# soedinglab/metaeuk

Hardware: AMD Instinct MI355X
Metric: prefilter+align ORF-fragments/sec (hits UNVERIFIED in this run: no CPU reference digest) (higher is better)
Workload: dtype packed i16 / i32 DP on u8 residues, i8 scores

## Files before the change

### metaeuk_amd/csrc/mk_align.hip

```cpp
#include "mk_align.hpp"
#include "mk_filters.hpp"
#include "mk_kernels.hpp"
#include "mk_limits.hpp"
#include "mk_segsort.hpp"
#include <algorithm>
#include <cmath>
#include <cstdlib>
#include <cstring>
#include <atomic>
#include <map>
#include <mutex>
#include <omp.h>

namespace mk {

namespace {

constexpr uint32_t KEY_CLS = 4096;
constexpr int SW_NBINCFG = SW_NCFG + 2;
constexpr uint32_t N_BINS = (uint32_t) SW_NBINCFG * KEY_CLS;
static_assert(SW_NCFG <= 16, "the bounds arrays keep 16 slots per kind");

__device__ __forceinline__ uint32_t len_class(uint32_t tLen) { return KEY_CLS - 1 - min(tLen >> 4, KEY_CLS - 1); }
__device__ __forceinline__ uint32_t sort_key(uint32_t qLen, uint32_t tLen) { return (uint32_t) sw_cfg_of(qLen) * KEY_CLS + len_class(tLen); }
// ... 41 lines not shown
    }
}

__global__ __launch_bounds__(256) void expand_pairs_kernel(AlignView V, const uint64_t *hitOff, const mk_hit *hits, uint64_t n,
                                                           SwJob *jobs, uint32_t *badTarget,
                                                           unsigned long long *work ) {
    helper_prio();
    __shared__ unsigned long long sWork[2 * SW_NCFG];
    for (int k = threadIdx.x; k < 2 * SW_NCFG; k += blockDim.x) sWork[k] = 0;
    __syncthreads();
    const uint64_t p = (uint64_t) blockIdx.x * blockDim.x + threadIdx.x;
    if (p < n) {
        uint32_t lo = 0, hi = V.n_queries;
        while (hi - lo > 1) { const uint32_t mid = (lo + hi) >> 1; if (hitOff[mid] <= p) lo = mid; else hi = mid; }
        const uint32_t q = lo, t = hits[p].seq_id;
        SwJob j;
        j.q_start = (uint32_t) V.q_off[q]; j.q_len = (uint32_t) (V.q_off[q + 1] - V.q_off[q]);
        if (t < V.n_targets) { j.t_start = V.t_off[t]; j.t_len = (uint32_t) (V.t_off[t + 1] - V.t_off[t]); }
        else { j.t_start = 0; j.t_len = 0; atomicMax(badTarget, (uint32_t) p + 1u); }
        j.q_step = 1; j.t_step = 1; j.slot = (uint32_t) p;
        jobs[p] = j;
        const int c = sw_cfg_of(j.q_len);
        atomicAdd(&sWork[2 * c], (unsigned long long) (j.t_len + 2u * j.q_len + (uint32_t) (sizeof(SwJob) + sizeof(SwOut))));
        atomicAdd(&sWork[2 * c + 1], (unsigned long long) j.q_len * j.t_len);
    }
    __syncthreads();
    for (int k = threadIdx.x; k < 2 * SW_NCFG; k += blockDim.x) if (sWork[k]) atomicAdd(&work[k], sWork[k]);
}

constexpr uint32_t ORDER_WAVE_MAX = 64, ORDER_TILE = 2048;
constexpr int PLAN_NV = 2 * SW_NCFG + 1;
constexpr uint32_t PLAN_BLOCK = 256;
struct PlanArgs {
    const uint64_t *hitOff; const uint64_t *q_off; uint32_t nq, nPairs; bool narrow;
    uint32_t *jobOff, *waveOff;
    uint32_t *runQuery, *runIndex;
    uint32_t *blockSums;
    uint32_t *bounds;
    uint32_t *waveStart;
};
__device__ __forceinline__ void plan_values(const PlanArgs &A, uint32_t q, uint32_t (&v)[PLAN_NV], int &cfg, uint32_t &n) {
#pragma unroll
    for (int k = 0; k < PLAN_NV; k++) v[k] = 0;
    cfg = 0; n = 0;
    if (q >= A.nq) return;
    n = (uint32_t) (A.hitOff[q + 1] - A.hitOff[q]);
    if (n == 0) return;
    cfg = sw_cfg_of((uint32_t) (A.q_off[q + 1] - A.q_off[q]));
    const uint32_t dpw = sw_cfg_jobs_per_wave(cfg, A.narrow);
#pragma unroll
    for (int c = 0; c < SW_NCFG; c++) if (c == cfg) { v[2 * c] = n; v[2 * c + 1] = (n + dpw - 1u) / dpw; }
    v[2 * SW_NCFG] = n > ORDER_WAVE_MAX ? (n + ORDER_TILE - 1u) / ORDER_TILE : 0u;
}
__global__ __launch_bounds__(PLAN_BLOCK) void plan_sums_kernel(PlanArgs A) {
    helper_prio();
    __shared__ uint32_t sm[PLAN_NV * 16];
    uint32_t v[PLAN_NV], excl[PLAN_NV], total[PLAN_NV], n;
    int cfg;
    plan_values(A, blockIdx.x * PLAN_BLOCK + threadIdx.x, v, cfg, n);
    segsort::block_scan<PLAN_NV>(v, excl, total, sm);
    if (threadIdx.x == 0)
#pragma unroll
        for (int k = 0; k < PLAN_NV; k++) A.blockSums[blockIdx.x * (PLAN_NV + 1) + k] = total[k];
}
__global__ __launch_bounds__(PLAN_BLOCK) void plan_offsets_kernel(PlanArgs A) {
    helper_prio();
    __shared__ uint32_t sm[PLAN_NV * 16];
    uint32_t v[PLAN_NV], w[PLAN_NV], excl[PLAN_NV], base[PLAN_NV], all[PLAN_NV], total[PLAN_NV], n;
#pragma unroll
    for (int k = 0; k < PLAN_NV; k++) { v[k] = 0; w[k] = 0; }
    for (uint32_t b = threadIdx.x; b < gridDim.x; b += PLAN_BLOCK)
#pragma unroll
        for (int k = 0; k < PLAN_NV; k++) {
            const uint32_t x = A.blockSums[b * (PLAN_NV + 1) + k];
            if (b < blockIdx.x) v[k] += x;
            w[k] += x;
        }
    segsort::block_scan<PLAN_NV>(v, excl, base, sm);
    segsort::block_scan<PLAN_NV>(w, excl, all, sm);
    const uint32_t q = blockIdx.x * PLAN_BLOCK + threadIdx.x;
    int cfg;
    plan_values(A, q, v, cfg, n);
    segsort::block_scan<PLAN_NV>(v, excl, total, sm);
    uint32_t jobBase = 0, waveBase = 0;
#pragma unroll
    for (int c = 0; c < SW_NCFG; c++) if (c < cfg) { jobBase += all[2 * c]; waveBase += all[2 * c + 1]; }
    if (q < A.nq) {
        uint32_t jo = jobBase, wo = waveBase;
#pragma unroll
        for (int c = 0; c < SW_NCFG; c++) if (c == cfg) { jo += base[2 * c] + excl[2 * c]; wo += base[2 * c + 1] + excl[2 * c + 1]; }
        A.jobOff[q] = jo; A.waveOff[q] = wo;
        const uint32_t runs = v[2 * SW_NCFG], r0 = base[2 * SW_NCFG] + excl[2 * SW_NCFG];
        for (uint32_t r = 0; r < runs; r++) { A.runQuery[r0 + r] = q; A.runIndex[r0 + r] = r; }
    }
    if (blockIdx.x == gridDim.x - 1 && threadIdx.x == 0) {
        uint32_t jb = 0, wb = 0;
        for (int c = 0; c < SW_NCFG; c++) { A.bounds[c] = jb; A.bounds[16 + c] = wb; jb += all[2 * c]; wb += all[2 * c + 1]; }
        A.bounds[SW_NCFG] = jb; A.bounds[16 + SW_NCFG] = wb; A.bounds[33] = all[2 * SW_NCFG];
        A.waveStart[wb] = A.nPairs;
    }
}
struct OrderArgs {
    const uint64_t *hitOff; const uint64_t *q_off; const mk_hit *hits; const uint64_t *t_off; uint32_t nq, nTargets; bool narrow;
    const uint32_t *jobOff, *waveOff, *runQuery, *runIndex;
    uint32_t *order, *waveStart;
};
__device__ __forceinline__ uint64_t order_key(const OrderArgs &A, uint64_t p) {
    const uint32_t t = A.hits[p].seq_id;
    const uint32_t tLen = t < A.nTargets ? (uint32_t) (A.t_off[t + 1] - A.t_off[t]) : 0u;
    return ((uint64_t) len_class(tLen) << 32) | (uint64_t) (uint32_t) p;
}
__global__ __launch_bounds__(256) void order_wave_kernel(OrderArgs A) {
    helper_prio();
    const uint32_t q = blockIdx.x * 4u + (threadIdx.x >> 6), lane = threadIdx.x & 63u;
    if (q >= A.nq) return;
    const uint64_t p0 = A.hitOff[q];
    const uint32_t n = (uint32_t) (A.hitOff[q + 1] - p0);
    if (n == 0 || n > ORDER_WAVE_MAX) return;
    const uint64_t key = lane < n ? order_key(A, p0 + lane) : ~0ull;
    const uint32_t r = segsort::wave_rank(key, n);
    const uint32_t jo = A.jobOff[q];
    if (lane < n) A.order[jo + r] = (uint32_t) (p0 + lane);
    const uint32_t dpw = sw_cfg_jobs_per_wave(sw_cfg_of((uint32_t) (A.q_off[q + 1] - A.q_off[q])), A.narrow);
    const uint32_t nW = (n + dpw - 1u) / dpw;
    if (lane < nW) A.waveStart[A.waveOff[q] + lane] = jo + lane * dpw;
}
__global__ __launch_bounds__(256) void order_block_kernel(OrderArgs A) {
    helper_prio();
    __shared__ uint64_t sK[ORDER_TILE];
    const uint32_t q = A.runQuery[blockIdx.x], run = A.runIndex[blockIdx.x];
    const uint64_t p0 = A.hitOff[q];
    const uint32_t n = (uint32_t) (A.hitOff[q + 1] - p0);
    const uint32_t b = run * ORDER_TILE, m = min(ORDER_TILE, n - b);
    const uint32_t P = segsort::pow2_at_least(m);
    for (uint32_t t = threadIdx.x; t < P; t += 256) sK[t] = t < m ? order_key(A, p0 + b + t) : ~0ull;
    __syncthreads();
    segsort::lds_sort<256>(sK, P);
    const uint32_t jo = A.jobOff[q] + b;
    for (uint32_t t = threadIdx.x; t < m; t += 256) A.order[jo + t] = (uint32_t) sK[t];
    const uint32_t dpw = sw_cfg_jobs_per_wave(sw_cfg_of((uint32_t) (A.q_off[q + 1] - A.q_off[q])), A.narrow);
    const uint32_t w0 = b / dpw, nW = (m + dpw - 1u) / dpw;
    for (uint32_t w = threadIdx.x; w < nW; w += 256) A.waveStart[A.waveOff[q] + w0 + w] = jo + w * dpw;
}
static_assert(ORDER_TILE % 8 == 0, "a run holds whole waves");

constexpr uint32_t SCAN_TILE = 1024;
__global__ __launch_bounds__(256) void scan_sums_kernel(const uint32_t *in, uint32_t n, uint32_t *blockSums) {
    helper_prio();
    __shared__ uint32_t sm[16];
    const uint32_t i0 = blockIdx.x * SCAN_TILE + threadIdx.x * 4u;
    uint32_t v[1] = {0}, excl[1], total[1];
#pragma unroll
    for (uint32_t k = 0; k < 4; k++) if (i0 + k < n) v[0] += in[i0 + k];
    segsort::block_scan<1>(v, excl, total, sm);
    if (threadIdx.x == 0) blockSums[blockIdx.x] = total[0];
}
__global__ __launch_bounds__(256) void scan_apply_kernel(const uint32_t *in, uint32_t n, uint32_t *out, const uint32_t *blockSums, uint32_t *grandTotal) {
    helper_prio();
    __shared__ uint32_t sm[16];
    uint32_t v[1] = {0}, excl[1], base[1], total[1];
    for (uint32_t b = threadIdx.x; b < blockIdx.x; b += 256) v[0] += blockSums[b];
    segsort::block_scan<1>(v, excl, base, sm);
    const uint32_t i0 = blockIdx.x * SCAN_TILE + threadIdx.x * 4u;
    uint32_t x[4];
    v[0] = 0;
#pragma unroll
    for (uint32_t k = 0; k < 4; k++) { x[k] = i0 + k < n ? in[i0 + k] : 0u; v[0] += x[k]; }
    segsort::block_scan<1>(v, excl, total, sm);
    uint32_t run = base[0] + excl[0];
#pragma unroll
    for (uint32_t k = 0; k < 4; k++) { if (i0 + k < n) out[i0 + k] = run; run += x[k]; }
    if (grandTotal && blockIdx.x == gridDim.x - 1 && threadIdx.x == 0) *grandTotal = base[0] + total[0];
}

__device__ __forceinline__ bool gate_pass(const SwJob *fwdJobs, const SwOut *fwdOut, uint64_t n, const GateEntry *gate, uint64_t p, SwJob &j) {
    if (p >= n) return false;
    const int score = fwdOut[p].score;
// ... 307 lines not shown
        for (int s = SCAN; s >= 1; s--) {
            const bool pass = !(eval(s) > evalThr);
            if (!pass) { lastFail = s; break; }
        }
        g.s0 = lastFail >= SCAN ? (1 << 30) : lastFail + 1;
        for (int s = 1; s < 256 && s < g.s0; s++)
            if (!(eval(s) > evalThr)) g.mask[s >> 5] |= 1u << (s & 31);
        table[L] = g;
    }
}

#define ACHK(x) do { hipError_t e_ = (x); if (e_ != hipSuccess) { err = std::string(#x) + ": " + hipGetErrorString(e_); return MK_ERR_DEVICE; } } while (0)
#define ANULL(p) do { if (!(p)) { err = "device scratch allocation failed (" #p ")"; return MK_ERR_DEVICE; } } while (0)

static int device_scan(const uint32_t *in, uint32_t n, uint32_t *out, uint32_t *total, hipStream_t stream, std::string &err) {
    if (n == 0) { if (total) ACHK(hipMemsetAsync(total, 0, 4, stream)); return MK_OK; }
    const uint32_t nb = (n + SCAN_TILE - 1u) / SCAN_TILE;
    uint32_t *sums = (uint32_t *) dev_scratch("align_scansums", (size_t) nb * 4);
    ANULL(sums);
    hipLaunchKernelGGL(scan_sums_kernel, dim3(nb), dim3(256), 0, stream, in, n, sums);
    hipLaunchKernelGGL(scan_apply_kernel, dim3(nb), dim3(256), 0, stream, in, n, out, (const uint32_t *) sums, total);
    ACHK(hipGetLastError());
    return MK_OK;
}

struct AlignShapes {
    int cus = 256;
    uint32_t persistentBlocks[SW_NCFG];
    uint32_t unitsPerBlock = 0;
    int knownForce = -1, knownWaves = 12;
    bool fwdLargeFirst = false;
    bool multiLargeFirst = true;
    bool multiPrio = true;
    uint32_t multiPerCu[3] = {24, 12, 12};
};
static bool sw_early_exit() { return knob_long("MK_SW_EARLY_EXIT", 1) != 0; }
static const AlignShapes &align_shapes() {
    static AlignShapes S;
    static std::once_flag once;
    std::call_once(once, [] {
        int dev = 0;
        (void) hipGetDevice(&dev);
        if (hipDeviceGetAttribute(&S.cus, hipDeviceAttributeMultiprocessorCount, dev) != hipSuccess || S.cus <= 0) S.cus = 256;
        int perCu[SW_NCFG];
        for (int c = 0; c < SW_NCFG; c++) perCu[c] = 12;
        if (const char *e = knob("MK_SW_WAVES_PER_CU")) {
            int k = 0, last = 16;
            for (const char *p = e; *p && k < SW_NCFG; k++) {
                last = std::max(1, atoi(p));
                perCu[k] = last;
                while (*p && *p != ',') p++;
                if (*p == ',') p++;
            }
            for (; k < SW_NCFG; k++) perCu[k] = last;
        }
        for (int c = 0; c < SW_NCFG; c++) S.persistentBlocks[c] = (uint32_t) (S.cus * perCu[c]);
        S.unitsPerBlock = (uint32_t) std::max(0L, knob_long("MK_SW_UNITS_PER_BLOCK", 0));
        S.knownForce = (int) knob_long("MK_SW_KNOWN", -1);
        S.knownWaves = (int) std::max(1L, knob_long("MK_SW_KNOWN_WAVES", 12));
        S.multiPrio = knob_long("MK_SW_MULTI_PRIO", 1) != 0;
        S.fwdLargeFirst = knob_long("MK_SW_FWD_LARGE_FIRST", 0) != 0;
        S.multiLargeFirst = knob_long("MK_SW_MULTI_LARGE_FIRST", 1) != 0;
        if (const char *e = knob("MK_SW_MULTI_WAVES")) {
            int k = 0;
            for (const char *p = e; *p && k < 3; k++) { S.multiPerCu[k] = (uint32_t) std::max(1, atoi(p)); while (*p && *p != ',') p++; if (*p == ',') p++; }
        }
    });
    return S;
}

static int tpos_first_cfg(const AlignView &V) {
    static_assert(SW_NCFG == 11, "configurations 8 / 9 = 512 / 768 rows");
    if (!V.q_prof || knob_long("MK_SW_TPOS", 1) == 0 || knob_long("MK_SW_MULTI", 0) != 0 || knob_long("MK_SW_NARROW", -1) == 0) return -1;
    return 8;
}

static int run_sorted_sw(const AlignView &V, const mk_params &P, const SwJob *jobs, SwOut *out, const uint32_t *keys, uint32_t *hist, uint32_t *order,
                         uint32_t n, const char *tag, hipStream_t stream, std::string &err,
                         timed_begin_fn tb, timed_end_fn te, int *handles ,
                         const int32_t *knownScore ) {
    if (handles) for (int c = 0; c < SW_NCFG; c++) handles[c] = -1;
    if (n == 0) return MK_OK;
    const AlignShapes &S = align_shapes();
    uint32_t *dCursor = (uint32_t *) dev_scratch("align_bincursor", (size_t) N_BINS * 4);
    uint32_t *dBounds = (uint32_t *) dev_scratch("align_bounds", 64 * sizeof(uint32_t));
    uint32_t *hb = (uint32_t *) pinned_scratch("align_bounds_h", 64 * sizeof(uint32_t));
    ANULL(dCursor); ANULL(dBounds); ANULL(hb);
    int th = tb("align_sort", 12.0 * n, 0);
    hipLaunchKernelGGL(bin_scan_kernel, dim3(1), dim3(BIN_THREADS), 0, stream, hist, dCursor, dBounds);
    hipLaunchKernelGGL(bin_scatter_kernel, dim3((n + 255) / 256), dim3(256), 0, stream, keys, n, dCursor, order);
// ... 70 lines not shown
        L.q_res = V.q_res; L.q_bias8 = V.q_bias8; L.q_prof = V.q_prof; L.t_res = V.t_res; L.mat = V.mat_aln;
        L.jobs = jobs; L.out = out; L.n_jobs = hi - lo; L.order = order + lo;
        L.boundary = nullptr; L.boundary_stride = 0; L.boundary_job0 = 0;
        L.wave_start = nullptr; L.n_waves = 0; L.work_counter = nullptr; L.persistent_blocks = 0; L.units_per_block = 0; L.known_score = knownScore;
        L.gap_open = P.gap_open; L.gap_extend = P.gap_extend;
        const int rows = sw_cfg_rows(8 + pc);
        char nm[64];
        snprintf(nm, sizeof(nm), "%s_rows%dt", tag, rows);
        th = tb(nm, 0, 0);
        ACHK(launch_sw_tpos(L, rows, (uint32_t) S.cus * (uint32_t) std::max(1L, knob_long("MK_SW_TPOS_WAVES", 32)), stream));
        te(th);
    }
    return MK_OK;
}

static int run_shared_fwd(const AlignView &V, const mk_params &P, const uint64_t *dHitOff, const mk_hit *dHits, const SwJob *jobs, SwOut *out,
                          uint32_t n, hipStream_t stream, std::string &err, timed_begin_fn tb, timed_end_fn te, int *handles ) {
    for (int c = 0; c < SW_NCFG; c++) handles[c] = -1;
    if (n == 0) return MK_OK;
    const AlignShapes &S = align_shapes();
    const uint32_t nq = V.n_queries;
    const uint32_t nb = (nq + PLAN_BLOCK - 1u) / PLAN_BLOCK;
    const uint32_t maxRuns = n / ORDER_TILE + nq + 1;
    uint32_t *dOrder = (uint32_t *) dev_scratch("align_order", (size_t) n * 4);
    uint32_t *dWave = (uint32_t *) dev_scratch("align_wavestart", ((size_t) n + 1) * 4);
    uint32_t *dPlan = (uint32_t *) dev_scratch("align_plan", ((size_t) nq * 2 + (size_t) maxRuns * 2 + (size_t) nb * (PLAN_NV + 1)) * 4);
    uint32_t *dBounds = (uint32_t *) dev_scratch("align_bounds", 64 * sizeof(uint32_t));
    uint32_t *hb = (uint32_t *) pinned_scratch("align_bounds_h", 64 * sizeof(uint32_t));
    uint32_t *dWork = (uint32_t *) dev_scratch("align_workcounters", 256);
    ANULL(dOrder); ANULL(dWave); ANULL(dPlan); ANULL(dBounds); ANULL(hb); ANULL(dWork);
    ACHK(hipMemsetAsync(dWork, 0, 256, stream));
    const long narrowForce = knob_long("MK_SW_NARROW", -1);
    const bool narrow = narrowForce >= 0 ? narrowForce != 0 : V.q_prof != nullptr;
    PlanArgs A;
    A.hitOff = dHitOff; A.q_off = V.q_off; A.nq = nq; A.nPairs = n; A.narrow = narrow;
    A.jobOff = dPlan; A.waveOff = dPlan + nq; A.runQuery = dPlan + 2 * (size_t) nq; A.runIndex = A.runQuery + maxRuns; A.blockSums = A.runIndex + maxRuns;
    A.bounds = dBounds; A.waveStart = dWave;
    int th = tb("align_sort", 24.0 * n, 0);
    hipLaunchKernelGGL(plan_sums_kernel, dim3(nb), dim3(PLAN_BLOCK), 0, stream, A);
    hipLaunchKernelGGL(plan_offsets_kernel, dim3(nb), dim3(PLAN_BLOCK), 0, stream, A);
    ACHK(hipGetLastError());
    ACHK(hipMemcpyAsync(hb, dBounds, 64 * sizeof(uint32_t), hipMemcpyDeviceToHost, stream));
    OrderArgs O;
    O.hitOff = dHitOff; O.q_off = V.q_off; O.hits = dHits; O.t_off = V.t_off; O.nq = nq; O.nTargets = V.n_targets; O.narrow = narrow;
    O.jobOff = A.jobOff; O.waveOff = A.waveOff; O.runQuery = A.runQuery; O.runIndex = A.runIndex; O.order = dOrder; O.waveStart = dWave;
    hipLaunchKernelGGL(order_wave_kernel, dim3((nq + 3) / 4), dim3(256), 0, stream, O);
    ACHK(hipGetLastError());
    ACHK(sync_wait(stream, "wait_align"));
    if (hb[33] > 0) {
        hipLaunchKernelGGL(order_block_kernel, dim3(hb[33]), dim3(256), 0, stream, O);
        ACHK(hipGetLastError());
    }
    te(th);
    for (int cc = 0; cc < SW_NCFG; cc++) {
        const int c = S.fwdLargeFirst ? SW_NCFG - 1 - cc : cc;
        const uint32_t lo = hb[c], hi = hb[c + 1], wlo = hb[16 + c], whi = hb[16 + c + 1];
        if (hi <= lo || whi <= wlo) continue;
        SwLaunch L;
        L.q_res = V.q_res; L.q_bias8 = V.q_bias8; L.q_prof = V.q_prof; L.t_res = V.t_res; L.mat = V.mat_aln;
        L.jobs = jobs; L.out = out; L.n_jobs = hi - lo; L.order = dOrder;
        L.boundary = nullptr; L.boundary_stride = 0; L.boundary_job0 = lo;
        L.wave_start = dWave + wlo; L.n_waves = whi - wlo;
        L.work_counter = dWork + c; L.work_counter_t = dWork + 16 + c; L.persistent_blocks = S.persistentBlocks[c]; L.units_per_block = S.unitsPerBlock;
        L.gap_open = P.gap_open; L.gap_extend = P.gap_extend;
        L.narrow = narrow;
        {
            static const long tMax = knob_long("MK_SW_T_MAXROWS", 256), tMinCfg = knob_long("MK_SW_T_MINCFG", 512);
            L.t_max_rows = (narrow && V.q_prof && sw_cfg_packed(c) && sw_cfg_rows(c) >= (int) tMinCfg) ? (uint32_t) std::max(0L, std::min(256L, tMax)) : 0u;
        }
        L.known_score = nullptr;
        if (c == SW_NCFG - 1 && V.max_q_len > (uint32_t) sw_cfg_rows(c)) {
            const uint32_t stride = V.max_t_len;
            L.boundary = (uint32_t *) dev_scratch("align_border", (size_t) (hi - lo) * stride * sizeof(uint32_t));
            ANULL(L.boundary);
            L.boundary_stride = stride;
        }
        char nm[64];
        snprintf(nm, sizeof(nm), "sw_fwd_rows%d", sw_cfg_rows(c));
        th = tb(nm, 0, 0);
        handles[c] = th;
        if (sw_cfg_packed(c)) ACHK(launch_sw_score(L, c, stream));
        else ACHK(launch_sw(L, c, stream));
        te(th);
    }
    return MK_OK;
}

static void set_range_work(const int *handles, const unsigned long long *work , timed_set_fn ts) {
    for (int c = 0; c < SW_NCFG; c++) {
        if (handles[c] < 0) continue;
        double bytes = 0, cells = 0;
        for (int k = c; k < SW_NCFG && (k == c || handles[k] < 0); k++) { bytes += (double) work[2 * k]; cells += (double) work[2 * k + 1]; }
        ts(handles[c], bytes, cells);
    }
}

int run_align_device(const AlignView &V, const uint64_t *hitOffHost, const mk_hit *hitsHost, uint64_t nPairs,
                     const std::vector<GateEntry> &gate, const mk_params &P, hipStream_t stream,
// ... 380 lines not shown
```

### metaeuk_amd/csrc/mk_kernels.hpp

```cpp
#pragma once
#include <hip/hip_runtime.h>
#include <cstdint>

namespace mk {

struct SwJob {
    uint64_t t_start;
    uint32_t q_start;
    uint32_t q_len;
    uint32_t t_len;
    int32_t q_step;
    int32_t t_step;
    uint32_t slot;
};
struct SwOut { int32_t score; int32_t end_col; int32_t end_row; int32_t pad; };

struct SwLaunch {
    const uint8_t *q_res; const int8_t *q_bias8;
    const int8_t *q_prof = nullptr;
    const uint8_t *t_res;
    const int8_t *mat;
    const SwJob *jobs; SwOut *out; uint64_t n_jobs;
    const uint32_t *order;
    uint32_t *boundary;
    uint32_t boundary_stride;
    int gap_open, gap_extend;
    const uint32_t *wave_start; uint64_t n_waves;
    uint32_t *work_counter;
    uint32_t *work_counter_t = nullptr;
    uint32_t t_max_rows = 0;
    uint32_t persistent_blocks;
    uint32_t units_per_block;
    uint64_t boundary_job0;
    const int32_t *known_score;
    bool narrow = false;
};

constexpr int SW_NCFG = 11;
__host__ __device__ inline int sw_cfg_rows(int c) {
    const int rows[SW_NCFG] = {32, 48, 64, 96, 128, 192, 256, 384, 512, 768, 1024};
    return rows[c];
}
__host__ __device__ inline bool sw_cfg_packed(int c) { return sw_cfg_rows(c) <= 768; }
__host__ __device__ inline uint32_t sw_cfg_jobs_per_wave(int c, bool narrow = false) {
    const int rows = sw_cfg_rows(c);
    return rows <= 256 ? 8u : (rows <= 768 ? (narrow ? 8u : 4u) : 1u);
}
__host__ __device__ inline int sw_cfg_of(uint32_t qLen) {
    int c = 0;
    while (c < SW_NCFG - 1 && (uint32_t) sw_cfg_rows(c) < qLen) c++;
    return c;
}
hipError_t launch_sw(const SwLaunch &L, int cfg, hipStream_t stream);
hipError_t launch_sw_score(const SwLaunch &L, int cfg, hipStream_t stream);
__host__ __device__ inline bool sw_cfg_known(int c) { return sw_cfg_rows(c) <= 64; }
hipError_t launch_sw_known(const SwLaunch &L, int cfg, hipStream_t stream);
constexpr uint32_t SW_TPOS_MAX_ROWS = 256;
hipError_t launch_sw_tpos(const SwLaunch &L, int rows, uint32_t blocksPerClass, hipStream_t stream);
hipError_t launch_sw_multi(const SwLaunch &L, const uint32_t *bounds, uint32_t *counter, int cls, uint32_t blocks, hipStream_t stream, bool prio = true);

template <class ScoreFn>
__host__ __device__ inline int ungapped_on_diagonal_fn(ScoreFn score_of, uint32_t qLen, const uint8_t *t, uint32_t tLen,
                                                       int diagonal, uint32_t minDist) {
    uint32_t len = 0, q0 = 0, t0 = 0;
    if (diagonal >= 0 && minDist < qLen) { len = tLen < qLen - minDist ? tLen : qLen - minDist; q0 = minDist; }
    else if (diagonal < 0 && minDist < tLen) { len = tLen - minDist < qLen ? tLen - minDist : qLen; t0 = minDist; }
    int score = 0, best = 0;
    for (uint32_t k = 0; k < len; k++) {
        const int curr = score_of(q0 + k, (uint32_t) t[t0 + k]);
        score = score + curr > 0 ? score + curr : 0;
        best = best > score ? best : score;
    }
    return best;
}
template <class ScoreFn>
__host__ __device__ inline int ungapped_score_fn(ScoreFn score_of, uint32_t qLen, const uint8_t *t, uint32_t tLen, uint32_t d16) {
    if (qLen >= 32768u || tLen >= 32768u) {
        int best = 0;
// ... 67 lines not shown
```

### metaeuk_amd/csrc/mk_sw.hip

```cpp
#include "mk_kernels.hpp"
#include <algorithm>
#include <mutex>

namespace mk {

template <int G>
__device__ __forceinline__ uint32_t shift_up(uint32_t top, uint32_t x, int laneInGroup) {
    if constexpr (G == 16) {
        return (uint32_t) __builtin_amdgcn_update_dpp((int) top, (int) x, 0x111 , 0xf, 0xf, false);
    } else if constexpr (G == 64) {
        return (uint32_t) __builtin_amdgcn_update_dpp((int) top, (int) x, 0x138 , 0xf, 0xf, false);
    } else {
        const uint32_t v = (uint32_t) __builtin_amdgcn_update_dpp((int) top, (int) x, 0x138 , 0xf, 0xf, false);
        return laneInGroup == 0 ? top : v;
    }
}

template <int G>
__device__ __forceinline__ uint32_t shift_up_zero(uint32_t x, int laneInGroup) {
    if constexpr (G == 16) return (uint32_t) __builtin_amdgcn_update_dpp((int) x, (int) x, 0x111 , 0xf, 0xf, true);
    else return shift_up<G>(0u, x, laneInGroup);
}

__device__ __forceinline__ int max3i(int a, int b, int c) { return max(max(a, b), c); }
// ... 665 lines not shown
                    H[r] = h;
                }
                hupPrev = hup;
                outH = pk_bits(H[R - 1]);
                outF = pk_bits(F);
                outRes = tres;
            }
            const uint32_t rose = pk_bits(best) ^ bestIn;
            if (rose & 0xFFFFu) roseA = s0;
            if (rose >> 16) roseB = s0;
        }
        uint32_t b = pk_bits(best);
#pragma unroll
        for (int m = G / 2; m >= 1; m >>= 1) b = pk_bits(pk_max(pk_from(b), pk_from((uint32_t) __shfl_xor((int) b, m, G))));
        uint32_t cA = (pk_bits(best) & 0xFFFFu) == (b & 0xFFFFu) ? (uint32_t) max(roseA + 15 - lane, 0) : 0x7FFFFFFFu;
        uint32_t cB = (pk_bits(best) >> 16) == (b >> 16) ? (uint32_t) max(roseB + 15 - lane, 0) : 0x7FFFFFFFu;
#pragma unroll
        for (int m = G / 2; m >= 1; m >>= 1) {
            cA = min(cA, (uint32_t) __shfl_xor((int) cA, m, G));
            cB = min(cB, (uint32_t) __shfl_xor((int) cB, m, G));
        }
        if (lane == 0) {
            SwOut o;
            o.end_row = -1; o.pad = 0;
            if (haveA) { o.score = (int32_t) (int16_t) (b & 0xFFFFu); o.end_col = (int32_t) min(cA, (uint32_t) lastA); L.out[jobA.slot] = o; }
            if (haveB) { o.score = (int32_t) (int16_t) (b >> 16); o.end_col = (int32_t) min(cB, (uint32_t) lastB); L.out[jobB.slot] = o; }
        }
        __builtin_amdgcn_fence(__ATOMIC_ACQ_REL, "wavefront");
        __builtin_amdgcn_wave_barrier();
        }
    }
}

template <int R, int RP>
__global__ __launch_bounds__(64) void swq_kernel(SwLaunch L) {
    constexpr int G = 16, ROWS = G * RP, NDP = 8;
    static_assert(RP >= R && RP % 2 == 0 && G * R * 127 <= 32767, "small tiles only");
    extern __shared__ __attribute__((aligned(16))) int8_t smem[];
    int16_t *prof = reinterpret_cast<int16_t *>(smem);
    constexpr int PROF1 = 22 * ROWS;
    int8_t *sMat = smem + (size_t) NDP * PROF1 * sizeof(int16_t);
    uint8_t *sQ = reinterpret_cast<uint8_t *>(sMat + 448);
    int8_t *sB = reinterpret_cast<int8_t *>(sQ + NDP * ROWS);
    for (int k = (int) threadIdx.x; k < 441; k += 64) sMat[k] = L.mat[k];
    const int lane = threadIdx.x % G, grp = threadIdx.x / G;
    const pk16 go2 = pk_splat(L.gap_open), ge2 = pk_splat(L.gap_extend), zero2 = pk_splat(0);
    const uint64_t nUnits = (L.n_jobs + NDP - 1) / NDP;
    for (;;) {
        uint32_t u = 0;
        if (threadIdx.x == 0) u = atomicAdd(L.work_counter, 1u);
        u = (uint32_t) __builtin_amdgcn_readfirstlane((int) u);
        if ((uint64_t) u >= nUnits) break;
        const uint64_t j0 = (uint64_t) u * NDP;
        const uint64_t ja = j0 + 2 * grp, jb = ja + 1;
        const bool haveA = ja < L.n_jobs, haveB = jb < L.n_jobs;
        const SwJob jobA = L.jobs[L.order[haveA ? ja : j0]], jobB = L.jobs[L.order[haveB ? jb : j0]];
        const int tLenA = haveA ? (int) jobA.t_len : 0, tLenB = haveB ? (int) jobB.t_len : 0;
        const uint32_t SA = haveA ? (uint32_t) L.known_score[jobA.slot] & 0xFFFFu : 0xFFFFu, SB = haveB ? (uint32_t) L.known_score[jobB.slot] & 0xFFFFu : 0xFFFFu;
        const uint32_t S2 = SA | (SB << 16);
        for (int i = (int) threadIdx.x; i < NDP * ROWS; i += 64) {
            const int dp = i / ROWS, slot = i - dp * ROWS;
            const uint64_t j = j0 + (uint64_t) dp;
            uint8_t qc = 255; int8_t bc = 0;
            if (j < L.n_jobs) {
                const SwJob jj = L.jobs[L.order[j]];
                const int row = RP == R ? slot : (slot / RP) * R + slot % RP;
// ... 105 lines not shown
}

hipError_t launch_sw_known(const SwLaunch &L, int cfg, hipStream_t stream) {
    if (!L.order || !L.work_counter || !L.known_score || cfg < 0 || cfg >= SW_NCFG || !sw_cfg_known(cfg)) return hipErrorInvalidValue;
    if (L.n_jobs == 0) return hipSuccess;
    const uint64_t nUnits = (L.n_jobs + 7) / 8;
    const uint64_t grid = std::min<uint64_t>(nUnits, L.persistent_blocks ? L.persistent_blocks : nUnits);
    const int rows = sw_cfg_rows(cfg);
    const size_t prows = rows == 48 ? 64 : rows;
    const size_t lds = (size_t) 8 * 22 * prows * sizeof(int16_t) + 448 + 2 * 8 * prows;
    switch (rows) {
        case 32: hipLaunchKernelGGL((swq_kernel<2, 2>), dim3((unsigned) grid), dim3(64), lds, stream, L); break;
        case 48: hipLaunchKernelGGL((swq_kernel<3, 4>), dim3((unsigned) grid), dim3(64), lds, stream, L); break;
        case 64: hipLaunchKernelGGL((swq_kernel<4, 4>), dim3((unsigned) grid), dim3(64), lds, stream, L); break;
        default: return hipErrorInvalidValue;
    }
    return hipGetLastError();
}

hipError_t launch_sw_score(const SwLaunch &L, int cfg, hipStream_t stream) {
    if (!L.wave_start || !L.work_counter || !L.order || cfg < 0 || cfg >= SW_NCFG || !sw_cfg_packed(cfg)) return hipErrorInvalidValue;
    if (L.n_waves == 0) return hipSuccess;
    const uint64_t grid = L.units_per_block ? (L.n_waves + L.units_per_block - 1) / L.units_per_block
                                            : std::min<uint64_t>(L.n_waves, L.persistent_blocks ? L.persistent_blocks : L.n_waves);
    const int rows = sw_cfg_rows(cfg);
    const size_t prows = rows == 48 ? 64 : rows;
    const size_t lds = (size_t) 22 * prows * sizeof(int16_t) + 448 + 2 * prows;
    if (L.t_max_rows) {
        if (!L.work_counter_t || !L.q_prof || !L.narrow || L.t_max_rows > SWT_MAX_ROWS) return hipErrorInvalidValue;
        hipLaunchKernelGGL(swt_kernel<0>, dim3((unsigned) grid), dim3(64), swt_image_bytes(rows), stream, L);
        if (L.t_max_rows > 64u) hipLaunchKernelGGL(swt_kernel<1>, dim3((unsigned) grid), dim3(64), swt_image_bytes(rows), stream, L);
        if (L.t_max_rows > 128u) hipLaunchKernelGGL(swt_kernel<2>, dim3((unsigned) grid), dim3(64), swt_image_bytes(rows), stream, L);
    }
    switch (rows) {
        case 32: hipLaunchKernelGGL((swp_kernel<2>), dim3((unsigned) grid), dim3(64), lds, stream, L); break;
        case 48: hipLaunchKernelGGL((swp_kernel<3, 4>), dim3((unsigned) grid), dim3(64), lds, stream, L); break;
        case 64: hipLaunchKernelGGL((swp_kernel<4>), dim3((unsigned) grid), dim3(64), lds, stream, L); break;
        case 96: hipLaunchKernelGGL((swp_kernel<6>), dim3((unsigned) grid), dim3(64), lds, stream, L); break;
        case 128: hipLaunchKernelGGL((swp_kernel<8>), dim3((unsigned) grid), dim3(64), lds, stream, L); break;
        case 192: hipLaunchKernelGGL((swp_kernel<12>), dim3((unsigned) grid), dim3(64), lds, stream, L); break;
        case 256: hipLaunchKernelGGL((swp_kernel<16>), dim3((unsigned) grid), dim3(64), lds, stream, L); break;
        case 384: if (L.narrow) hipLaunchKernelGGL((swp_kernel<24, 24, 16>), dim3((unsigned) grid), dim3(64), lds, stream, L);
                  else hipLaunchKernelGGL((swp_kernel<12, 12, 32>), dim3((unsigned) grid), dim3(64), lds, stream, L);
                  break;
        case 512: hipLaunchKernelGGL((swp_kernel<16, 16, 32>), dim3((unsigned) grid), dim3(64), lds, stream, L); break;
        case 768: hipLaunchKernelGGL((swp_kernel<24, 24, 32>), dim3((unsigned) grid), dim3(64), lds, stream, L); break;
        default: return hipErrorInvalidValue;
    }
    return hipGetLastError();
}

hipError_t launch_sw_tpos(const SwLaunch &L, int rows, uint32_t blocksPerClass, hipStream_t stream) {
    if (!L.q_prof || !L.order || !L.known_score || rows <= 0) return hipErrorInvalidValue;
    if (L.n_jobs == 0) return hipSuccess;
    const unsigned grid = (unsigned) std::min<uint64_t>((L.n_jobs + 7) / 8, std::max<uint32_t>(1u, blocksPerClass));
    hipLaunchKernelGGL(swtp_kernel<0>, dim3(grid), dim3(64), swt_image_bytes(rows), stream, L);
    hipLaunchKernelGGL(swtp_kernel<1>, dim3(grid), dim3(64), swt_image_bytes(rows), stream, L);
    hipLaunchKernelGGL(swtp_kernel<2>, dim3(grid), dim3(64), swt_image_bytes(rows), stream, L);
    return hipGetLastError();
}

template <int G, int R, int BLOCK>
static hipError_t launch_one(const SwLaunch &L, hipStream_t stream) {
    if (L.wave_start) {
        const size_t lds = (size_t) 24 * G * R;
        if (L.n_waves == 0) return hipSuccess;
// ... 61 lines not shown
```

Baseline: 2.541 million.

## Add streaming SW kernel processing query-sharing job units per 16-lane group

Adds a new swps_kernel for the three smallest query configs. Each 16-lane group pulls a unit of 64 jobs that share one query, builds that query's profile once, and streams target pairs through it, prefetching the next jobs and residues. The planner and order kernels now size waves by this stream unit instead of 8 jobs. The aim is to reuse the query profile and cut per-wave setup and atomics, at the cost of coarser work units, which may worsen load balance, plus an added code path selected by knobs.

```diff
diff --git a/metaeuk_amd/csrc/mk_align.hip b/metaeuk_amd/csrc/mk_align.hip
--- a/metaeuk_amd/csrc/mk_align.hip
+++ b/metaeuk_amd/csrc/mk_align.hip
@@ -97,7 +97,7 @@
 constexpr int PLAN_NV = 2 * SW_NCFG + 1;
 constexpr uint32_t PLAN_BLOCK = 256;
 struct PlanArgs {
-    const uint64_t *hitOff; const uint64_t *q_off; uint32_t nq, nPairs; bool narrow;
+    const uint64_t *hitOff; const uint64_t *q_off; uint32_t nq, nPairs; bool narrow; uint32_t stream, streamUnit;
     uint32_t *jobOff, *waveOff;
     uint32_t *runQuery, *runIndex;
     uint32_t *blockSums;
@@ -112,7 +112,7 @@
     n = (uint32_t) (A.hitOff[q + 1] - A.hitOff[q]);
     if (n == 0) return;
     cfg = sw_cfg_of((uint32_t) (A.q_off[q + 1] - A.q_off[q]));
-    const uint32_t dpw = sw_cfg_jobs_per_wave(cfg, A.narrow);
+    const uint32_t dpw = sw_cfg_jobs_per_wave(cfg, A.narrow, A.stream, A.streamUnit);
 #pragma unroll
     for (int c = 0; c < SW_NCFG; c++) if (c == cfg) { v[2 * c] = n; v[2 * c + 1] = (n + dpw - 1u) / dpw; }
     v[2 * SW_NCFG] = n > ORDER_WAVE_MAX ? (n + ORDER_TILE - 1u) / ORDER_TILE : 0u;
@@ -166,7 +166,7 @@
     }
 }
 struct OrderArgs {
-    const uint64_t *hitOff; const uint64_t *q_off; const mk_hit *hits; const uint64_t *t_off; uint32_t nq, nTargets; bool narrow;
+    const uint64_t *hitOff; const uint64_t *q_off; const mk_hit *hits; const uint64_t *t_off; uint32_t nq, nTargets; bool narrow; uint32_t stream, streamUnit;
     const uint32_t *jobOff, *waveOff, *runQuery, *runIndex;
     uint32_t *order, *waveStart;
 };
@@ -186,7 +186,7 @@
     const uint32_t r = segsort::wave_rank(key, n);
     const uint32_t jo = A.jobOff[q];
     if (lane < n) A.order[jo + r] = (uint32_t) (p0 + lane);
-    const uint32_t dpw = sw_cfg_jobs_per_wave(sw_cfg_of((uint32_t) (A.q_off[q + 1] - A.q_off[q])), A.narrow);
+    const uint32_t dpw = sw_cfg_jobs_per_wave(sw_cfg_of((uint32_t) (A.q_off[q + 1] - A.q_off[q])), A.narrow, A.stream, A.streamUnit);
     const uint32_t nW = (n + dpw - 1u) / dpw;
     if (lane < nW) A.waveStart[A.waveOff[q] + lane] = jo + lane * dpw;
 }
@@ -203,11 +203,11 @@
     segsort::lds_sort<256>(sK, P);
     const uint32_t jo = A.jobOff[q] + b;
     for (uint32_t t = threadIdx.x; t < m; t += 256) A.order[jo + t] = (uint32_t) sK[t];
-    const uint32_t dpw = sw_cfg_jobs_per_wave(sw_cfg_of((uint32_t) (A.q_off[q + 1] - A.q_off[q])), A.narrow);
+    const uint32_t dpw = sw_cfg_jobs_per_wave(sw_cfg_of((uint32_t) (A.q_off[q + 1] - A.q_off[q])), A.narrow, A.stream, A.streamUnit);
     const uint32_t w0 = b / dpw, nW = (m + dpw - 1u) / dpw;
     for (uint32_t w = threadIdx.x; w < nW; w += 256) A.waveStart[A.waveOff[q] + w0 + w] = jo + w * dpw;
 }
-static_assert(ORDER_TILE % 8 == 0, "a run holds whole waves");
+static_assert(ORDER_TILE % 8 == 0 && ORDER_TILE % SW_STREAM_UNIT == 0 && SW_STREAM_UNIT % 2 == 0, "a run holds whole waves / units, a unit whole pairs");
 
 constexpr uint32_t SCAN_TILE = 1024;
 __global__ __launch_bounds__(256) void scan_sums_kernel(const uint32_t *in, uint32_t n, uint32_t *blockSums) {
@@ -581,6 +581,8 @@
     bool fwdLargeFirst = false;
     bool multiLargeFirst = true;
     bool multiPrio = true;
+    uint32_t streamCfgs = SW_STREAM_CFGS;
+    uint32_t streamUnit = SW_STREAM_UNIT;
     uint32_t multiPerCu[3] = {24, 12, 12};
 };
 static bool sw_early_exit() { return knob_long("MK_SW_EARLY_EXIT", 1) != 0; }
@@ -605,6 +607,9 @@
         }
         for (int c = 0; c < SW_NCFG; c++) S.persistentBlocks[c] = (uint32_t) (S.cus * perCu[c]);
         S.unitsPerBlock = (uint32_t) std::max(0L, knob_long("MK_SW_UNITS_PER_BLOCK", 0));
+        S.streamCfgs = (uint32_t) knob_long("MK_SW_STREAM", (long) S.streamCfgs) & SW_STREAM_CFGS;
+        for (uint32_t unit = 2; unit <= ORDER_TILE; unit *= 2)
+            if ((long) unit == knob_long("MK_SW_STREAM_UNIT", (long) SW_STREAM_UNIT)) S.streamUnit = unit;
         S.knownForce = (int) knob_long("MK_SW_KNOWN", -1);
         S.knownWaves = (int) std::max(1L, knob_long("MK_SW_KNOWN_WAVES", 12));
         S.multiPrio = knob_long("MK_SW_MULTI_PRIO", 1) != 0;
@@ -741,8 +746,9 @@
     ACHK(hipMemsetAsync(dWork, 0, 256, stream));
     const long narrowForce = knob_long("MK_SW_NARROW", -1);
     const bool narrow = narrowForce >= 0 ? narrowForce != 0 : V.q_prof != nullptr;
+    const uint32_t streamCfgs = (narrow || V.q_prof) ? 0u : S.streamCfgs;
     PlanArgs A;
-    A.hitOff = dHitOff; A.q_off = V.q_off; A.nq = nq; A.nPairs = n; A.narrow = narrow;
+    A.hitOff = dHitOff; A.q_off = V.q_off; A.nq = nq; A.nPairs = n; A.narrow = narrow; A.stream = streamCfgs; A.streamUnit = S.streamUnit;
     A.jobOff = dPlan; A.waveOff = dPlan + nq; A.runQuery = dPlan + 2 * (size_t) nq; A.runIndex = A.runQuery + maxRuns; A.blockSums = A.runIndex + maxRuns;
     A.bounds = dBounds; A.waveStart = dWave;
     int th = tb("align_sort", 24.0 * n, 0);
@@ -751,7 +757,7 @@
     ACHK(hipGetLastError());
     ACHK(hipMemcpyAsync(hb, dBounds, 64 * sizeof(uint32_t), hipMemcpyDeviceToHost, stream));
     OrderArgs O;
-    O.hitOff = dHitOff; O.q_off = V.q_off; O.hits = dHits; O.t_off = V.t_off; O.nq = nq; O.nTargets = V.n_targets; O.narrow = narrow;
+    O.hitOff = dHitOff; O.q_off = V.q_off; O.hits = dHits; O.t_off = V.t_off; O.nq = nq; O.nTargets = V.n_targets; O.narrow = narrow; O.stream = streamCfgs; O.streamUnit = S.streamUnit;
     O.jobOff = A.jobOff; O.waveOff = A.waveOff; O.runQuery = A.runQuery; O.runIndex = A.runIndex; O.order = dOrder; O.waveStart = dWave;
     hipLaunchKernelGGL(order_wave_kernel, dim3((nq + 3) / 4), dim3(256), 0, stream, O);
     ACHK(hipGetLastError());
@@ -773,6 +779,7 @@
         L.work_counter = dWork + c; L.work_counter_t = dWork + 16 + c; L.persistent_blocks = S.persistentBlocks[c]; L.units_per_block = S.unitsPerBlock;
         L.gap_open = P.gap_open; L.gap_extend = P.gap_extend;
         L.narrow = narrow;
+        L.stream = (streamCfgs >> c & 1u) != 0;
         {
             static const long tMax = knob_long("MK_SW_T_MAXROWS", 256), tMinCfg = knob_long("MK_SW_T_MINCFG", 512);
             L.t_max_rows = (narrow && V.q_prof && sw_cfg_packed(c) && sw_cfg_rows(c) >= (int) tMinCfg) ? (uint32_t) std::max(0L, std::min(256L, tMax)) : 0u;
diff --git a/metaeuk_amd/csrc/mk_kernels.hpp b/metaeuk_amd/csrc/mk_kernels.hpp
--- a/metaeuk_amd/csrc/mk_kernels.hpp
+++ b/metaeuk_amd/csrc/mk_kernels.hpp
@@ -34,6 +34,7 @@
     uint64_t boundary_job0;
     const int32_t *known_score;
     bool narrow = false;
+    bool stream = false;
 };
 
 constexpr int SW_NCFG = 11;
@@ -42,8 +43,11 @@
     return rows[c];
 }
 __host__ __device__ inline bool sw_cfg_packed(int c) { return sw_cfg_rows(c) <= 768; }
-__host__ __device__ inline uint32_t sw_cfg_jobs_per_wave(int c, bool narrow = false) {
+constexpr uint32_t SW_STREAM_CFGS = 0x7u;
+constexpr uint32_t SW_STREAM_UNIT = 64;
+__host__ __device__ inline uint32_t sw_cfg_jobs_per_wave(int c, bool narrow = false, uint32_t stream = 0, uint32_t streamUnit = SW_STREAM_UNIT) {
     const int rows = sw_cfg_rows(c);
+    if (!narrow && ((stream & SW_STREAM_CFGS) >> c & 1u)) return streamUnit;
     return rows <= 256 ? 8u : (rows <= 768 ? (narrow ? 8u : 4u) : 1u);
 }
 __host__ __device__ inline int sw_cfg_of(uint32_t qLen) {
diff --git a/metaeuk_amd/csrc/mk_sw.hip b/metaeuk_amd/csrc/mk_sw.hip
--- a/metaeuk_amd/csrc/mk_sw.hip
+++ b/metaeuk_amd/csrc/mk_sw.hip
@@ -721,6 +721,202 @@
     }
 }
 
+template <int CTRL>
+__device__ __forceinline__ uint32_t row_xchg(uint32_t x) { return (uint32_t) __builtin_amdgcn_update_dpp((int) x, (int) x, CTRL, 0xf, 0xf, false); }
+__device__ __forceinline__ uint32_t row_pk_max(uint32_t b) {
+    b = pk_bits(pk_max(pk_from(b), pk_from(row_xchg<0xB1>(b))));
+    b = pk_bits(pk_max(pk_from(b), pk_from(row_xchg<0x4E>(b))));
+    b = pk_bits(pk_max(pk_from(b), pk_from(row_xchg<0x141>(b))));
+    return pk_bits(pk_max(pk_from(b), pk_from(row_xchg<0x140>(b))));
+}
+__device__ __forceinline__ uint32_t row_min(uint32_t c) {
+    c = min(c, row_xchg<0xB1>(c));
+    c = min(c, row_xchg<0x4E>(c));
+    c = min(c, row_xchg<0x141>(c));
+    return min(c, row_xchg<0x140>(c));
+}
+__device__ __forceinline__ void wave_sync_lds() {
+    __builtin_amdgcn_fence(__ATOMIC_ACQ_REL, "wavefront");
+    asm volatile("s_waitcnt lgkmcnt(0)" ::: "memory");
+    __builtin_amdgcn_wave_barrier();
+}
+
+__host__ __device__ constexpr int swps_profile_entries(int rows) { return 22 * rows + (rows % 64 == 0 ? 64 : 0); }
+
+template <int R, int RP = R>
+__global__ __launch_bounds__(64) void swps_kernel(SwLaunch L) {
+    constexpr int G = 16, ROWS = G * RP, PROF1 = swps_profile_entries(ROWS);
+    static_assert(RP >= R && RP % 2 == 0 && G * R * 127 <= 32767, "small tiles only: no saturation");
+    extern __shared__ __attribute__((aligned(16))) int8_t smem[];
+    int8_t *sMat = smem + (size_t) 4 * PROF1 * sizeof(int16_t);
+    for (int k = (int) threadIdx.x; k < 441; k += 64) sMat[k] = L.mat[k];
+    wave_sync_lds();
+    const int lane = threadIdx.x % G, grp = threadIdx.x / G;
+    int16_t *prof = reinterpret_cast<int16_t *>(smem) + (size_t) grp * PROF1;
+    const char *profLane = reinterpret_cast<const char *>(prof + lane * RP);
+    const pk16 go2 = pk_splat(L.gap_open), ge2 = pk_splat(L.gap_extend), zero2 = pk_splat(0);
+    constexpr uint32_t ROWB = (uint32_t) ROWS * 2u, NOCOL = 21u * ROWB | (21u * ROWB) << 16;
+
+    pk16 H[R], E[R];
+#pragma unroll
+    for (int r = 0; r < R; r++) { H[r] = zero2; E[r] = zero2; }
+    pk16 best = zero2, hupPrev = zero2;
+    int roseA = 0, roseB = 0;
+    uint32_t outH = 0, outF = 0, outRes = NOCOL;
+    uint32_t tq0 = NOCOL, tq1 = NOCOL, tq2 = NOCOL;
+    int tLenA = 0, tLenB = 0, lastA = 0, lastB = 0;
+    int64_t baseA = 0, baseB = 0, stepA = 1, stepB = 1;
+    uint32_t slotA = 0, slotB = 0;
+    bool haveB = false;
+    int s0 = 0, steps = 0;
+    uint32_t p = 0, pEnd = 0, iA = 0, iB = 0, pulled = 0;
+    SwJob nA = {}, nB = {};
+    bool active = false, need = true;
+
+    const auto residue_a = [&](int col) -> uint32_t { return L.t_res[baseA + (int64_t) min(col, lastA) * stepA]; };
+    const auto residue_b = [&](int col) -> uint32_t { return L.t_res[baseB + (int64_t) min(col, lastB) * stepB]; };
+    const auto offsets = [&](int col, uint32_t va, uint32_t vb) -> uint32_t {
+        const uint32_t ra = col < tLenA ? va : 21u, rb = col < tLenB ? vb : 21u;
+        return ra * ROWB | (rb * ROWB) << 16;
+    };
+    const auto fetch = [&](int col) -> uint32_t { return offsets(col, residue_a(col), residue_b(col)); };
+
+    for (;;) {
+        if (need) {
+            if (active) {
+                const uint32_t b = row_pk_max(pk_bits(best));
+                uint32_t cA = (pk_bits(best) & 0xFFFFu) == (b & 0xFFFFu) ? (uint32_t) max(roseA + 15 - lane, 0) : 0x7FFFFFFFu;
+                uint32_t cB = (pk_bits(best) >> 16) == (b >> 16) ? (uint32_t) max(roseB + 15 - lane, 0) : 0x7FFFFFFFu;
+                cA = row_min(cA);
+                cB = row_min(cB);
+                if (lane == 0) {
+                    SwOut o;
+                    o.end_row = -1; o.pad = 0;
+                    o.score = (int32_t) (int16_t) (b & 0xFFFFu); o.end_col = (int32_t) min(cA, (uint32_t) lastA); L.out[slotA] = o;
+                    if (haveB) { o.score = (int32_t) (int16_t) (b >> 16); o.end_col = (int32_t) min(cB, (uint32_t) lastB); L.out[slotB] = o; }
+                }
+            }
+            bool work = true;
+            if (!active || p + 2u >= pEnd) {
+                uint32_t u = 0xFFFFFFFFu;
+                if (L.units_per_block == 0 || pulled < L.units_per_block) {
+                    if (lane == 0) u = atomicAdd(L.work_counter, 1u);
+                    u = (uint32_t) __shfl((int) u, 0, G);
+                    pulled++;
+                }
+                work = (uint64_t) u < L.n_waves;
+                if (work) {
+                    const uint32_t w0 = L.wave_start[u];
+                    pEnd = L.wave_start[u + 1];
+                    iA = L.order[w0]; iB = L.order[min(w0 + 1u, pEnd - 1u)];
+                    nA = L.jobs[iA]; nB = L.jobs[iB];
+                    iA = L.order[min(w0 + 2u, pEnd - 1u)]; iB = L.order[min(w0 + 3u, pEnd - 1u)];
+                    p = w0 - 2u;
+                    const int qLen = (int) nA.q_len;
+                    uint32_t qc[RP];
+                    int qb[RP];
+                    bool real[RP];
+#pragma unroll
+                    for (int k = 0; k < RP; k++) {
+                        const int row = lane * R + k;
+                        real[k] = k < R && row < qLen;
+                        const int64_t qi = qLen > 0 ? (int64_t) nA.q_start + (int64_t) (real[k] ? row : 0) * nA.q_step : 0;
+                        qc[k] = L.q_res[qi];
+                        qb[k] = L.q_bias8[qi];
+                    }
+                    uint32_t *pw = reinterpret_cast<uint32_t *>(prof + lane * RP);
+#pragma unroll 7
+                    for (int t = 0; t < 21; t++) {
+#pragma unroll
+                        for (int k = 0; k < RP; k += 2) {
+                            const int mlo = sMat[t * 21 + (int) qc[k]], mhi = sMat[t * 21 + (int) qc[k + 1]];
+                            const int lo = real[k] ? mlo + qb[k] : 0, hi = real[k + 1] ? mhi + qb[k + 1] : 0;
+                            pw[(t * ROWS + k) / 2] = ((uint32_t) lo & 0xFFFFu) | ((uint32_t) hi << 16);
+                        }
+                    }
+#pragma unroll
+                    for (int k = 0; k < RP; k += 2) pw[(21 * ROWS + k) / 2] = 0u;
+                    wave_sync_lds();
+                }
+            }
+            if (work) {
+                p += 2u;
+                haveB = p + 1u < pEnd;
+                tLenA = (int) nA.t_len; tLenB = haveB ? (int) nB.t_len : 0;
+                baseA = tLenA > 0 ? (int64_t) nA.t_start : 0; stepA = nA.t_step; slotA = nA.slot;
+                baseB = tLenB > 0 ? (int64_t) nB.t_start : 0; stepB = nB.t_step; slotB = nB.slot;
+                lastA = max(tLenA - 1, 0); lastB = max(tLenB - 1, 0);
+                steps = max((max(tLenA, tLenB) + G - 1 + 15) & ~15, 16);
+                s0 = 0;
+                nA = L.jobs[iA]; nB = L.jobs[iB];
+                iA = L.order[min(p + 4u, pEnd - 1u)]; iB = L.order[min(p + 5u, pEnd - 1u)];
+                tq0 = fetch(lane); tq1 = fetch(16 + lane); tq2 = fetch(32 + lane);
+            } else {
+                tLenA = 0; tLenB = 0;
+                tq0 = NOCOL; tq1 = NOCOL; tq2 = NOCOL;
+            }
+#pragma unroll
+            for (int r = 0; r < R; r++) { H[r] = zero2; E[r] = zero2; }
+            best = zero2; hupPrev = zero2;
+            roseA = 0; roseB = 0;
+            outH = 0; outF = 0; outRes = NOCOL;
+            active = work;
+            need = false;
+        }
+        if (__builtin_amdgcn_ballot_w64(active) == 0ull) break;
+
+        uint32_t tcur = tq0;
+        tq0 = tq1; tq1 = tq2;
+        const int colAhead = s0 + 48 + lane;
+        const uint32_t aheadA = residue_a(colAhead), aheadB = residue_b(colAhead);
+        const uint32_t bestIn = pk_bits(best);
+#pragma unroll
+        for (int k = 0; k < 16; k++) {
+            const uint32_t top = tcur;
+            tcur = (uint32_t) __builtin_amdgcn_update_dpp(0, (int) tcur, 0x12F , 0xf, 0xf, false);
+            const pk16 hup = pk_from(shift_up_zero<G>(outH, lane));
+            pk16 F = pk_from(shift_up_zero<G>(outF, lane));
+            const uint32_t tres = shift_up<G>(top, outRes, lane);
+            const int16_t *pa = reinterpret_cast<const int16_t *>(profLane + (tres & 0xFFFFu)), *pb = reinterpret_cast<const int16_t *>(profLane + (tres >> 16));
+            uint32_t wa[RP / 2], wb[RP / 2];
+            if constexpr (RP % 4 == 0) {
+                const uint64_t *qa = reinterpret_cast<const uint64_t *>(__builtin_assume_aligned(pa, 8)), *qb = reinterpret_cast<const uint64_t *>(__builtin_assume_aligned(pb, 8));
+#pragma unroll
+                for (int k = 0; k < RP / 4; k++) {
+                    const uint64_t xa = qa[k], xb = qb[k];
+                    wa[2 * k] = (uint32_t) xa; wa[2 * k + 1] = (uint32_t) (xa >> 32); wb[2 * k] = (uint32_t) xb; wb[2 * k + 1] = (uint32_t) (xb >> 32);
+                }
+            } else {
+#pragma unroll
+                for (int k = 0; k < RP / 2; k++) { wa[k] = reinterpret_cast<const uint32_t *>(pa)[k]; wb[k] = reinterpret_cast<const uint32_t *>(pb)[k]; }
+            }
+            pk16 dsave = hupPrev;
+#pragma unroll
+            for (int r = 0; r < R; r++) {
+                const pk16 sc = pk_from(__builtin_amdgcn_perm(wb[r / 2], wa[r / 2], (r & 1) ? 0x07060302u : 0x05040100u));
+                const pk16 d = dsave + sc;
+                dsave = H[r];
+                const pk16 h = pk_max(pk_max(d, E[r]), F);
+                best = pk_max(best, h);
+                const pk16 ho = pk_subs0(h, go2);
+                E[r] = pk_max(pk_subs0(E[r], ge2), ho);
+                F = pk_max(pk_subs0(F, ge2), ho);
+                H[r] = h;
+            }
+            hupPrev = hup;
+            outH = pk_bits(H[R - 1]);
+            outF = pk_bits(F);
+            outRes = tres;
+        }
+        const uint32_t rose = pk_bits(best) ^ bestIn;
+        if (rose & 0xFFFFu) roseA = s0;
+        if (rose >> 16) roseB = s0;
+        tq2 = offsets(colAhead, aheadA, aheadB);
+        s0 += 16;
+        need = active && s0 >= steps;
+    }
+}
+
 template <int R, int RP>
 __global__ __launch_bounds__(64) void swq_kernel(SwLaunch L) {
     constexpr int G = 16, ROWS = G * RP, NDP = 8;
@@ -892,6 +1088,16 @@
         if (L.t_max_rows > 64u) hipLaunchKernelGGL(swt_kernel<1>, dim3((unsigned) grid), dim3(64), swt_image_bytes(rows), stream, L);
         if (L.t_max_rows > 128u) hipLaunchKernelGGL(swt_kernel<2>, dim3((unsigned) grid), dim3(64), swt_image_bytes(rows), stream, L);
     }
+    if (L.stream) {
+        if (rows > 64 || L.q_prof || L.narrow || L.t_max_rows) return hipErrorInvalidValue;
+        const size_t ldsStream = (size_t) 4 * swps_profile_entries((int) prows) * sizeof(int16_t) + 448;
+        switch (rows) {
+            case 32: hipLaunchKernelGGL((swps_kernel<2>), dim3((unsigned) grid), dim3(64), ldsStream, stream, L); break;
+            case 48: hipLaunchKernelGGL((swps_kernel<3, 4>), dim3((unsigned) grid), dim3(64), ldsStream, stream, L); break;
+            default: hipLaunchKernelGGL((swps_kernel<4>), dim3((unsigned) grid), dim3(64), ldsStream, stream, L); break;
+        }
+        return hipGetLastError();
+    }
     switch (rows) {
         case 32: hipLaunchKernelGGL((swp_kernel<2>), dim3((unsigned) grid), dim3(64), lds, stream, L); break;
         case 48: hipLaunchKernelGGL((swp_kernel<3, 4>), dim3((unsigned) grid), dim3(64), lds, stream, L); break;
```

Result: slower. 2.396 million (-5.7%).
